# lrm2017/Fastest_Image_Pattern_Matching

Measured on AMD Instinct MI355X. Metric: template matches/sec + ms/search, 4024×3036 src ±180°; HBM GB/s vs roofline, higher is better.
Workload: dtype u8

## Files before the change

### fastest_image_pattern_matching_amd/_lib.py

```python
from __future__ import annotations

import ctypes as C
import os
import subprocess

_HERE = os.path.dirname(os.path.abspath(__file__))
LIB_PATH = os.path.join(_HERE, "lib", "libfpm_hip.so")
CSRC = os.path.join(_HERE, "csrc")

FPM_OK = 0
FPM_E_INVALID_ARG = -1
FPM_E_NOT_LEARNED = -2
FPM_E_SIZE = -3
FPM_E_DEVICE = -4
FPM_E_CAPACITY = -5
FPM_E_INTERNAL = -6

(FMT_GRAY8, FMT_BGR8, FMT_RGB8, FMT_BGRA8, FMT_RGBA8, FMT_BGR8_PLANAR, FMT_RGB8_PLANAR) = range(7)
FMT_COUNT = 7

(K_PYR, K_TOP_WARP, K_TOP_NCC, K_TOP_NMS, K_CAND_INIT, K_ROI_TABLES, K_ROI_WARP, K_ROI_CORR, K_ROI_EVAL, K_ROI_SMALL,
 K_CAND_STEP, K_TOP_MAP, K_NOT, K_PATCH, K_COMPARE, K_LEARN) = range(16)
KERNEL_NAMES = ["pyr_down", "top_warp", "top_ncc", "top_nms", "cand_init", "roi_tables", "roi_warp", "roi_corr",
                "roi_eval", "roi_small", "cand_step", "top_map", "bitwise_not", "patch_warp", "patch_compare"]
# ... 84 lines not shown
class AlignResult(C.Structure):

    _fields_ = [("lt_x", C.c_float), ("lt_y", C.c_float), ("angle", C.c_double), ("ssd_start", C.c_int64),
                ("ssd", C.c_int64), ("n_used", C.c_int64), ("evals", C.c_int32), ("best_eval", C.c_int32),
                ("flags", C.c_int32), ("reserved", C.c_int32)]


class Blob(C.Structure):

    _fields_ = [(n, C.c_int32) for n in ("hit", "seed", "area", "x0", "y0", "x1", "y1", "max_value")] + \
               [(n, C.c_int64) for n in ("sum_value", "sum_x", "sum_y")]


class BlobSummary(C.Structure):

    _fields_ = [("fg_pixels", C.c_int64)] + \
               [(n, C.c_int32) for n in ("n_components", "n_blobs", "n_returned", "largest_area", "flags", "reserved")]


class RoiRecord(C.Structure):

    _fields_ = [("score", C.c_float), ("mx", C.c_int32), ("my", C.c_int32), ("on_border", C.c_int32),
                ("vec", C.c_float * 9)]


class Peak(C.Structure):

    _fields_ = [("x", C.c_int32), ("y", C.c_int32), ("score", C.c_float)]


PEAKS_STATS_CALL, PEAKS_STATS_JOB = 8, 4
PEAKS_RAN_BLOCKS, PEAKS_RAN_NMS, PEAKS_RAN_FAST, PEAKS_RAN_GREEDY = 1, 2, 4, 8
TOP_MAPS_STATS = 8
TOP_FUSED_STATS = 8
TOP_FORM_EXACT16, TOP_FORM_EXACT14, TOP_FORM_SMALL, TOP_FORM_LARGE = 0, 1, 2, 3

_P = C.c_void_p
_U8P = C.POINTER(C.c_uint8)
SIGNATURES = {
    "fpm_params_default": (None, [C.POINTER(Params)]),
    "fpm_abi_version": (C.c_int, []),
    "fpm_create": (C.c_int, [C.c_int, C.POINTER(_P)]),
    "fpm_destroy": (C.c_int, [_P]),
    "fpm_last_error": (C.c_char_p, [_P]),
    "fpm_set_params": (C.c_int, [_P, C.POINTER(Params)]),
    "fpm_get_params": (C.c_int, [_P, C.POINTER(Params)]),
    "fpm_learn": (C.c_int, [_P, _U8P, C.c_int32, C.c_int32, C.c_size_t]),
    "fpm_clear_pattern": (C.c_int, [_P]),
    "fpm_is_learned": (C.c_int, [_P]),
    "fpm_match": (C.c_int, [_P, _U8P, C.c_int32, C.c_int32, C.c_size_t, C.POINTER(Result), C.c_int32,
                            C.POINTER(C.c_int32), C.POINTER(C.c_double)]),
    "fpm_stage_sources": (C.c_int, [_P, C.POINTER(_U8P), C.c_int32, C.c_int32, C.c_int32, C.c_size_t]),
    "fpm_stage_sources_device": (C.c_int, [_P, C.POINTER(_P), C.c_int32, C.c_int32, C.c_int32, C.c_size_t, C.c_size_t,
                                           C.c_int32, _P]),
    "fpm_match_device": (C.c_int, [_P, _P, C.c_int32, C.c_int32, C.c_size_t, C.c_size_t, C.c_int32, _P,
                                   C.POINTER(Result), C.c_int32, C.POINTER(C.c_int32), C.POINTER(C.c_double)]),
    "fpm_match_staged": (C.c_int, [_P, C.POINTER(Result), C.c_int32, C.POINTER(C.c_int32)]),
    "fpm_match_staged_launch": (C.c_int, [_P]),
    "fpm_match_staged_finish": (C.c_int, [_P, C.POINTER(Result), C.c_int32, C.POINTER(C.c_int32)]),
    "fpm_op_pyr_down": (C.c_int, [_P, _U8P, C.c_int32, C.c_int32, C.c_size_t, _U8P, C.c_size_t]),
    "fpm_op_pyr_down2": (C.c_int, [_P, _U8P, C.c_int32, C.c_int32, C.c_size_t, _U8P, C.c_size_t, _U8P, C.c_size_t,
                                   C.c_int32, C.c_int32]),
    "fpm_op_bitwise_not": (C.c_int, [_P, _U8P, C.c_int32, C.c_int32, C.c_size_t, _U8P, C.c_size_t]),
    "fpm_op_to_gray": (C.c_int, [_P, _P, C.c_int32, C.c_int32, C.c_size_t, C.c_size_t, C.c_int32, C.c_int32, _U8P,
                                 C.c_size_t]),
    "fpm_op_warp_affine": (C.c_int, [_P, _U8P, C.c_int32, C.c_int32, C.c_size_t, C.POINTER(C.c_double), _U8P,
                                     C.c_int32, C.c_int32, C.c_size_t, C.c_int32]),
# ... 144 lines not shown
```

### fastest_image_pattern_matching_amd/csrc/fpm_engine.hip

```cpp
#include <hip/hip_runtime.h>

#include <algorithm>
#include <array>
#include <cfloat>
#include <chrono>
#include <cmath>
#include <cstddef>
#include <cstdio>
#include <cstdlib>
#include <cstring>
#include <new>
#include <random>
#include <string>
#include <vector>

#include "../../include/fpm.h"
#include "fpm_host.h"
#include "fpm_kernels.h"
#include "fpm_model.h"

using namespace fpm;

namespace {

// ... 753 lines not shown
    hipStream_t st = ctx->stream;
    const SrcLevel& top = ctx->src[L];
    const TmplLevel& tt = ctx->tmpl[L];
    {
        const int64_t bytes = (int64_t)P.nang * top.w * top.h;
        ProfScope ps(ctx, FPM_K_TOP_WARP, bytes * S);
        launch_warp(P.d_jobs.as<WarpJob>(P.off_warp), J, P.max_canvas, st, P.d_livecnt.as<int32_t>(), P.nzero);
    }
    {
        int64_t bytes = 0;
        for (int a = 0; a < P.nang; ++a) bytes += 4LL * P.map_w[a] * P.map_h[a];
        ProfScope ps(ctx, FPM_K_TOP_NCC, bytes * S);
        if (ncc_tile_fits(tt.w, tt.h)) {
            int mw = 0, mh = 0;
            for (int a = 0; a < P.nang; ++a) { mw = std::max(mw, P.map_w[a]); mh = std::max(mh, P.map_h[a]); }
            launch_ncc_tile(P.d_jobs.as<NccJob>(P.off_ncc), J, mw, mh, tt.w, tt.h, st);
        } else {
            launch_ncc_map(P.d_jobs.as<NccJob>(P.off_ncc), J, P.max_map, tt.w * tt.h, st);
        }
    }
}

size_t plan_top_fused_lds(const fpm_ctx* ctx, size_t* need = nullptr) {
    const Plan& P = ctx->plan;
    const TmplLevel& tt = ctx->tmpl[P.L];
    if (need) *need = 0;
    if (P.by_block || !ncc_tile_fits(tt.w, tt.h) || P.S * P.nang <= 0) return 0;
    size_t lds = 0;
    for (int a = 0; a < P.nang; ++a) lds = std::max(lds, top_fused_lds(P.top[a].bw, P.top[a].bh, tt.w, tt.h));
    if (need) *need = lds;
    return lds > top_fused_lds_limit() ? 0 : lds;
}

void plan_top_choice(const fpm_ctx* ctx, size_t* fused_lds, bool* use_mma) {
    const Plan& P = ctx->plan;
    const char* top_env = getenv("FPM_TOP_FUSED");
    const int top_mode = top_env ? atoi(top_env) : -1;
    *fused_lds = 0;
    if (top_mode != 0 && (P.S * P.nang >= kTopFusedMinJobs || top_mode == 1)) *fused_lds = plan_top_fused_lds(ctx);
    const char* mma_env = getenv("FPM_TOP_MMA");
    *use_mma = P.top_mma && (*fused_lds == 0 || (mma_env && atoi(mma_env) == 1));
    if (*use_mma) *fused_lds = 0;
}

NmsArgs plan_nms_args(const fpm_ctx* ctx) {
    const Plan& P = ctx->plan;
    const TmplLevel& tt = ctx->tmpl[P.L];
    NmsArgs na{};
    na.jobs = P.d_jobs.as<NmsJob>(P.off_nms);
    na.peaks = P.d_peaks.as<Peak>();
    na.counts = P.d_counts.as<int32_t>();
    na.tw = tt.w; na.th = tt.h; na.cap = P.cap; na.by_block = P.by_block ? 1 : 0;
    na.mfc = ctx->prm.semantics == FPM_SEMANTICS_MFC ? 1 : 0;
    na.thr = P.layer_score[P.L]; na.overlap = ctx->prm.max_overlap;
    na.lds_blocks = 0;
    na.cand = nullptr; na.cand_cnt = nullptr; na.cand_cap = 0; na.cand_lds = 0; na.stamps = nullptr;
    na.skey = nullptr; na.sdone = nullptr;
    return na;
}

int enqueue_search(fpm_ctx* ctx) {
    Plan& P = ctx->plan;
    const int L = P.L, S = P.S, J = S * P.nang;
    const int stop = P.stop;
    hipStream_t st = ctx->stream;
    uint8_t* dsrc = ctx->d_src.as<uint8_t>();
    const SrcLevel& top = ctx->src[L];
    P.step_layers = 0;
    P.top_lists = false;
    size_t fused_lds = 0;
    bool use_mma = false;
    plan_top_choice(ctx, &fused_lds, &use_mma);
    int32_t* live[2] = {P.d_live.as<int32_t>(), P.d_live.as<int32_t>() + P.C};
    int32_t* livecnt = P.d_livecnt.as<int32_t>();
    CandInitArgs ca;
    ca.peaks = P.d_peaks.as<Peak>();
    ca.counts = P.d_counts.as<int32_t>();
    ca.angles = P.d_top.as<TopAngle>();
    ca.top_nodes = P.d_topn.as<AngleNode>();
    ca.state = P.d_state.as<CandState>();
    ca.live = live[0];
    ca.live_count = livecnt + 0;
    ca.nang = P.nang; ca.cap = P.cap; ca.total = P.C;
    ca.center = P.center;
    ca.refine = L > stop ? (L - 1 == stop ? 2 : 1) : 0;
    bool cand_fused = false;
    const bool top_init = fused_lds > 0 && P.cap <= kNmsInitCap && (size_t)J * P.cap == (size_t)P.C;
    const bool pyr_zero = (top_init && L >= 1) || use_mma;
    enqueue_pyramid(ctx, pyr_zero);
    NmsArgs na = plan_nms_args(ctx);
    if (fused_lds > 0) {
        int64_t bytes = (int64_t)P.nang * top.w * top.h;
        for (int a = 0; a < P.nang; ++a) bytes += 4LL * P.map_w[a] * P.map_h[a];
        ProfScope ps(ctx, FPM_K_TOP_NCC, bytes * S);
        launch_top_fused(P.d_jobs.as<WarpJob>(P.off_warp), P.d_jobs.as<NccJob>(P.off_ncc), na, J, fused_lds,
                         pyr_zero ? nullptr : P.d_livecnt.as<int32_t>(), pyr_zero ? 0 : P.nzero, st,
                         top_init ? &ca : nullptr, P.d_jobs.as<int32_t>(P.off_order), false);
        cand_fused = top_init;
    }
    if (use_mma) {
        const int mdim = P.nmax.max_map_dim;
        const long mpx = P.nmax.max_map_px;
        TopMmaArgs ta = P.tma;
        {
            ProfScope ps(ctx, FPM_K_TOP_NCC, (int64_t)S * P.nang * top.w * top.h);
            ta.mode = 0;
            launch_top_mma(ta, st);
        }
        const bool ci_ok = !P.by_block && P.cap <= kNmsInitCap && (size_t)J * P.cap == (size_t)P.C;
        NmsArgs ga = na;
        ga.cand = P.d_ncand.as<int32_t>(); ga.cand_val = P.d_tcandv.as<float>();
        ga.cand_cnt = ta.cand_cnt; ga.cand_cap = P.tcand_cap;
        ga.reset_untaken = P.by_block ? 1 : 0;
        {
            ProfScope ps(ctx, FPM_K_TOP_NMS, 0);
            launch_top_greedy(ga, J, P.max_cells, st, ci_ok ? &ca : nullptr);
        }
        P.top_lists = true;
        {
            ProfScope ps(ctx, FPM_K_TOP_MAP, 0);
            ta.mode = 1;
            launch_top_mma(ta, st);
        }
        {
            ProfScope ps(ctx, FPM_K_TOP_NMS, 0);
            NmsArgs fa = na;
            fa.cand = ga.cand; fa.cand_cnt = ga.cand_cnt; fa.cand_cap = P.tcand_cap;
            if (P.by_block) {
                fa.skey = (uint64_t*)(P.d_livecnt.as<int32_t>() + P.off_skey);
                fa.sdone = P.d_livecnt.as<int32_t>() + P.off_skey + 6 * J;
// ... 3205 lines not shown

int fpm_op_top_fused(fpm_ctx* ctx, int32_t* n_sources, int32_t* n_angles, int64_t* map_floats, int32_t* cap,
                     int32_t* geom, int32_t geom_cap, float* maps, int64_t maps_cap, fpm_peak* peaks, int32_t* counts,
                     fpm_peak* dump_peaks, int32_t* dump_counts, int64_t peak_slots, int32_t* stats) {
    if (!ctx) return FPM_E_INVALID_ARG;
    if (!ctx->learned) { ctx->err = "template not learned"; return FPM_E_NOT_LEARNED; }
    if (ctx->pending) { ctx->err = "a search is in flight (fpm_match_staged_finish first)"; return FPM_E_INVALID_ARG; }
    if (ctx->S <= 0 || !ctx->staged || !ctx->src_valid) { ctx->err = "top fused: no staged sources"; return FPM_E_INVALID_ARG; }
    const bool sizing = !geom && !maps && !peaks && !counts && !dump_peaks && !dump_counts;
    if (geom_cap < 0 || maps_cap < 0 || peak_slots < 0 ||
        (!sizing && (!geom || !maps || !peaks || !counts || !dump_peaks || !dump_counts))) {
        ctx->err = "bad top fused arguments";
        return FPM_E_INVALID_ARG;
    }
    HIP_TRY(hipSetDevice(ctx->device));
    struct ProfOff {
        fpm_ctx* c; bool was;
        explicit ProfOff(fpm_ctx* x) : c(x), was(x->prof) { c->prof = false; }
        ~ProfOff() { c->prof = was; }
    } prof_off(ctx);
    int rc = build_plan(ctx);
    if (rc != FPM_OK) return rc;
    Plan& P = ctx->plan;
    const int S = P.S, nang = P.nang, J = S * nang;
    std::vector<size_t> dense_off(nang);
    size_t dense = 0;
    for (int a = 0; a < nang; ++a) { dense_off[a] = dense; dense += (size_t)P.map_w[a] * P.map_h[a]; }
    if (n_sources) *n_sources = S;
    if (n_angles) *n_angles = nang;
    if (map_floats) *map_floats = (int64_t)dense;
    if (cap) *cap = P.cap;
    size_t need = 0;
    const size_t lds = plan_top_fused_lds(ctx, &need);
    if (stats) {
        size_t chosen = 0;
        bool use_mma = false;
        plan_top_choice(ctx, &chosen, &use_mma);
        std::fill(stats, stats + FPM_TOP_FUSED_STATS, 0);
        stats[0] = (int32_t)need;
        stats[1] = (int32_t)top_fused_static_lds(false);
        stats[2] = (int32_t)top_fused_lds_limit();
        stats[3] = top_fused_grid(J);
        stats[4] = J;
        stats[5] = P.cap;
        stats[6] = chosen > 0 ? 1 : 0;
        stats[7] = (int32_t)top_fused_static_lds(true);
    }
    if (lds == 0 && J > 0) {
        ctx->err = "top fused: the plan cannot take the fused form (block mode, the template level or the LDS limit)";
        return FPM_E_SIZE;
    }
    if (sizing) return FPM_OK;
    const size_t slots = (size_t)J * P.cap;
    if (geom_cap < nang || (uint64_t)maps_cap < (uint64_t)dense * S || (uint64_t)peak_slots < (uint64_t)slots) {
        ctx->err = "top fused: output capacity below the sizing call's";
        return FPM_E_CAPACITY;
    }
    for (int a = 0; a < nang; ++a) {
        geom[4 * a + 0] = P.top[a].bw; geom[4 * a + 1] = P.top[a].bh;
        geom[4 * a + 2] = P.map_w[a]; geom[4 * a + 3] = P.map_h[a];
    }
    if (J <= 0) return FPM_OK;
    hipStream_t st = ctx->stream;
    const size_t o_peaks[2] = {0, round_up(sizeof(Peak) * slots, (size_t)256)};
    const size_t o_counts[2] = {2 * o_peaks[1], 2 * o_peaks[1] + round_up(sizeof(int32_t) * J, (size_t)256)};
    HIP_TRY(ctx->d_op_b.ensure(o_counts[1] + sizeof(int32_t) * J));
    fpm_peak* hp_out[2] = {peaks, dump_peaks};
    int32_t* hc_out[2] = {counts, dump_counts};
    std::vector<Peak> hp[2];
    for (int v = 0; v < 2; ++v) {
        hp[v].resize(slots);
        for (size_t k = 0; k < slots; ++k) {
            Peak& q = hp[v][k];
            q.x = hp_out[v][k].x; q.y = hp_out[v][k].y; q.score = hp_out[v][k].score; q.pad = 0;
        }
        HIP_TRY(hipMemcpyAsync(ctx->d_op_b.as<char>(o_peaks[v]), hp[v].data(), sizeof(Peak) * slots, hipMemcpyHostToDevice, st));
        HIP_TRY(hipMemcpyAsync(ctx->d_op_b.as<char>(o_counts[v]), hc_out[v], sizeof(int32_t) * J, hipMemcpyHostToDevice, st));
    }
    rc = apply_polarity(ctx);
    if (rc != FPM_OK) return rc;
    HIP_TRY(hipMemsetAsync(P.d_map.p, 0xff, sizeof(float) * P.map_floats * S, st));
    enqueue_pyramid(ctx, false);
    for (int v = 0; v < 2; ++v) {
        NmsArgs na = plan_nms_args(ctx);
        na.peaks = ctx->d_op_b.as<Peak>(o_peaks[v]);
        na.counts = ctx->d_op_b.as<int32_t>(o_counts[v]);
        launch_top_fused(P.d_jobs.as<WarpJob>(P.off_warp), P.d_jobs.as<NccJob>(P.off_ncc), na, J, lds,
                         P.d_livecnt.as<int32_t>(), P.nzero, st, nullptr, P.d_jobs.as<int32_t>(P.off_order), v == 1);
        HIP_TRY(hipGetLastError());
    }
    std::vector<float> hm(P.map_floats * S);
    HIP_TRY(hipMemcpyAsync(hm.data(), P.d_map.p, sizeof(float) * hm.size(), hipMemcpyDeviceToHost, st));
    for (int v = 0; v < 2; ++v) {
        HIP_TRY(hipMemcpyAsync(hp[v].data(), ctx->d_op_b.as<char>(o_peaks[v]), sizeof(Peak) * slots, hipMemcpyDeviceToHost, st));
        HIP_TRY(hipMemcpyAsync(hc_out[v], ctx->d_op_b.as<char>(o_counts[v]), sizeof(int32_t) * J, hipMemcpyDeviceToHost, st));
    }
    HIP_TRY(hipStreamSynchronize(st));
    for (int s = 0; s < S; ++s)
        for (int a = 0; a < nang; ++a)
            std::copy_n(hm.data() + P.map_floats * s + P.map_off[a], (size_t)P.map_w[a] * P.map_h[a],
                        maps + dense * s + dense_off[a]);
    for (int v = 0; v < 2; ++v)
        for (size_t k = 0; k < slots; ++k) {
            fpm_peak& p = hp_out[v][k];
            const Peak& q = hp[v][k];
            p.x = q.x; p.y = q.y; p.score = q.score;
        }
    return FPM_OK;
}

int fpm_profile_enable(fpm_ctx* ctx, int32_t enable) {
    if (!ctx) return FPM_E_INVALID_ARG;
    ctx->prof = enable != 0;
    return FPM_OK;
}

int fpm_profile_reset(fpm_ctx* ctx) {
    if (!ctx) return FPM_E_INVALID_ARG;
    for (auto& k : ctx->kp) { k.ms = 0; k.launches = 0; k.bytes = 0; k.used = 0; }
    return FPM_OK;
}
// ... 19 lines not shown
```

### fastest_image_pattern_matching_amd/csrc/fpm_kernels.h

```cpp
#pragma once
#include <hip/hip_runtime.h>
#include <stdint.h>

#include "fpm_geom.h"

namespace fpm {

struct WarpJob {
    const uint8_t* src;
    uint8_t* dst;
    int32_t sw, sh, sp;
    int32_t dw, dh, dp;
    int32_t border;
    int32_t pad;
    double M[6];
};

struct NccJob {
    const uint8_t* img;
    const uint8_t* tmpl;
    float* out;
    int32_t iw, ih, ip;
    int32_t tw, th, tp;
    int32_t ow, oh;
// ... 270 lines not shown
    uint64_t* acc;
    uint32_t slack_off;
    int32_t nlv, nchunks;
    TmplPrepLevel lv[kTmplPrepMaxLevels];
};
bool launch_tmpl_prep(const TmplPrepArgs& a, hipStream_t st);
void launch_ncc_map(const NccJob* jobs, int njobs, int max_out, int tmpl_bytes, hipStream_t st);
bool ncc_tile_fits(int tw, int th);
void launch_ncc_tile(const NccJob* jobs, int njobs, int max_ow, int max_oh, int tw, int th, hipStream_t st);
constexpr int kNmsCandCap = 8192;
constexpr int kNmsInitCap = 128;
enum { kNmsRanBlocks = 1, kNmsRanNms = 2, kNmsRanFast = 4, kNmsRanGreedy = 8 };
struct NmsLaunchInfo {
    uint32_t kernels;
    int32_t lds_blocks;
    int32_t cand_lds;
    int32_t greedy_cap;
    int32_t blk_lds;
};
void launch_nms(const NmsArgs& a, int njobs, int max_blocks, int max_map_dim, int max_cells, hipStream_t st,
                int max_items = 0, const CandInitArgs* ci = nullptr, long max_map_px = -1,
                NmsLaunchInfo* info = nullptr);
int nms_block_items(int mw, int mh, int tw, int th, int mfc);
struct NmsMaxima {
    int max_blocks = 0, max_map_dim = 0, max_cells = 0, max_items = 0;
    long max_map_px = 0;
};
int nms_maxima_add(NmsMaxima& m, int mw, int mh, int tw, int th, int by_block, int mfc);
int nms_plain_form(int blk_lds, int cap, long n);
void launch_cand_init(const CandInitArgs& a, hipStream_t st);
size_t top_fused_lds(int bw, int bh, int tw, int th);
size_t top_fused_lds_limit();
constexpr int kTopFusedMinJobs = 256;
void launch_top_fused(const WarpJob* wjobs, const NccJob* njobs, const NmsArgs& a, int njobs_n, size_t lds,
                      int32_t* zero, int nzero, hipStream_t st, const CandInitArgs* ci, const int32_t* order,
                      bool dump);
size_t top_fused_static_lds(bool dump);
int top_fused_grid(int njobs_n);
struct TopUnit { int32_t job, x0, y0, y1; };
constexpr int kTopMmaMaxSw = 192;
struct TopMmaArgs {
    const WarpJob* wjobs;
    const NccJob* njobs;
    const TopUnit* units;
    int32_t nunits;
    const uint8_t* bfrag;
    int32_t nq, R;
    int32_t tw, th, area;
    uint32_t tsum;
    int32_t sw;
    int32_t cp;
    int32_t rr;
    int32_t ct, rt;
    int32_t o_colt, o_rowt, o_bf, o_ft;
    int32_t nqm;
    int32_t mode;
    int32_t prefilter;
    float thrK, E;
    double thr, mean, norm, inv_area;
    int32_t* cand;
    float* cand_val;
    int32_t* cand_cnt;
    int32_t cand_cap;
};
size_t top_mma_lds(const TopMmaArgs& a);
void top_mma_layout(TopMmaArgs& a, int sw, int max_rows);
bool top_mma_fits(int tw, int th);
void launch_top_mma(const TopMmaArgs& a, hipStream_t st);
enum { kTopFormExact16 = 0, kTopFormExact14 = 1, kTopFormSmall = 2, kTopFormLarge = 3 };
// ... 29 lines not shown
```

### fastest_image_pattern_matching_amd/csrc/fpm_kernels.hip

```cpp
#include <float.h>
#include <stdio.h>
#include <stdlib.h>
#include <limits.h>

#include <map>
#include <mutex>
#include <type_traits>
#include <utility>

#include "../../include/fpm.h"
#include "fpm_kernels.h"
#include "fpm_model.h"
#include "fpm_rrect.h"

static void ensure_lds_attr(const void* fn, size_t bytes) {
    if (bytes <= 65536) return;
    int dev = 0;
    (void)hipGetDevice(&dev);
    static std::mutex mu;
    static std::map<std::pair<int, const void*>, size_t> done;
    std::lock_guard<std::mutex> lock(mu);
    size_t& cur = done[std::make_pair(dev, fn)];
    if (bytes <= cur) return;
    (void)hipFuncSetAttribute(fn, hipFuncAttributeMaxDynamicSharedMemorySize, (int)bytes);
// ... 5 lines not shown
__device__ __forceinline__ int rint_i(double v) { return (int)__builtin_rint(v); }
__device__ __forceinline__ int sat_s16(int v) { return v < -32768 ? -32768 : (v > 32767 ? 32767 : v); }
__device__ __forceinline__ int reflect101(int p, int n) {
    if (n == 1) return 0;
    while (p < 0 || p >= n) p = p < 0 ? -p : 2 * n - 2 - p;
    return p;
}
__device__ __forceinline__ double dmax0(double a) { return a < 0.0 ? 0.0 : a; }
__device__ __forceinline__ double dmin(double a, double b) { return b < a ? b : a; }

__device__ __forceinline__ int warp_tap(const uint8_t* __restrict__ src, int sw, int sh, int sp, int X, int Y,
                                        int cval) {
    const int sx = sat_s16(X >> kInterBits), sy = sat_s16(Y >> kInterBits);
    const int fx = X & (kInterTab - 1), fy = Y & (kInterTab - 1);
    const int w0 = (kInterTab - fy) * (kInterTab - fx) * 32, w1 = (kInterTab - fy) * fx * 32;
    const int w2 = fy * (kInterTab - fx) * 32, w3 = fy * fx * 32;
    int v0, v1, v2, v3;
    if ((unsigned)sx < (unsigned)(sw > 1 ? sw - 1 : 0) && (unsigned)sy < (unsigned)(sh > 1 ? sh - 1 : 0)) {
        const uint8_t* p = src + (size_t)sy * sp + sx;
        v0 = p[0]; v1 = p[1]; v2 = p[sp]; v3 = p[sp + 1];
    } else if (sx >= sw || sx + 1 < 0 || sy >= sh || sy + 1 < 0) {
        return cval;
    } else {
        const bool x0 = sx >= 0 && sx < sw, x1 = sx + 1 >= 0 && sx + 1 < sw;
        const bool y0 = sy >= 0 && sy < sh, y1 = sy + 1 >= 0 && sy + 1 < sh;
        const uint8_t* r0 = src + (size_t)sy * sp;
        const uint8_t* r1 = r0 + sp;
        v0 = x0 && y0 ? r0[sx] : cval;
        v1 = x1 && y0 ? r0[sx + 1] : cval;
        v2 = x0 && y1 ? r1[sx] : cval;
        v3 = x1 && y1 ? r1[sx + 1] : cval;
    }
    return (v0 * w0 + v1 * w1 + v2 * w2 + v3 * w3 + (1 << 14)) >> 15;
}

__device__ __forceinline__ float ccoeff(double num, double wsum, double wsq, double mean0, double tnorm,
                                        double inv_area) {
    double wndMean2 = 0, wndSum2 = 0, t;
    t = wsum;
    wndMean2 += t * t;
    num -= t * mean0;
    wndMean2 *= inv_area;
    t = wsq;
    wndSum2 += t;
    const double diff2 = dmax0(wndSum2 - wndMean2);
    if (diff2 <= dmin(0.5, (double)(10 * FLT_EPSILON) * wndSum2))
        t = 0;
    else
        t = __builtin_sqrt(diff2) * tnorm;
    if (__builtin_fabs(num) < t)
        num /= t;
    else if (__builtin_fabs(num) < t * 1.125)
        num = num > 0 ? 1 : -1;
    else
        num = 0;
    return (float)num;
}

__device__ __forceinline__ int xcd_remap(int b, int n) {
    const int q = n >> 3, r = n & 7, x = b & 7;
    return (x < r ? x * (q + 1) : r * (q + 1) + (x - r) * q) + (b >> 3);
}
struct XcdSplit { int lo, hi, k, nk; };
__device__ __forceinline__ XcdSplit xcd_split(int n) {
    const int G = gridDim.x, b = blockIdx.x, x = b & 7, q = G >> 3, r = G & 7;
    const int nk = q + (x < r ? 1 : 0);
// ... 1730 lines not shown
    const int job = id / a.cap, r = id - job * a.cap, ang = job % a.nang;
    CandState s;
    s.lt = f2(0.f, 0.f);
    s.node = ang;
    s.alive = 0;
    s.reached0 = 0;
    s.pad = 0;
    if (r < a.counts[job]) {
        const Peak pk = a.peaks[id];
        const F2 pt = f2((float)pk.x - a.angles[ang].tx, (float)pk.y - a.angles[ang].ty);
        s.lt = rotate_pt(pt, a.center, a.top_nodes[ang].cn, a.top_nodes[ang].sn);
        if (a.refine) {
            s.alive = 1;
            s.reached0 = mark_reached0;
            const int slot = atomicAdd(a.live_count, 1);
            a.live[slot] = id;
        }
    }
    a.state[id] = s;
}

void launch_cand_init(const CandInitArgs& a, hipStream_t st) {
    if (a.total <= 0) return;
    CandInitArgs b = a;
    const int mark = a.refine == 2 ? 1 : 0;
    if (b.refine) b.refine = 1;
    hipLaunchKernelGGL(k_cand_init, dim3((a.total + 255) / 256), dim3(256), 0, st, b, mark);
}

constexpr int kTopThreads = 256;
template <bool DUMP>
__device__ __forceinline__ void top_fused_job(int job, const WarpJob* __restrict__ wjobs,
                                              const NccJob* __restrict__ njobs, const NmsArgs& a,
                                              const CandInitArgs& ci, int ci_mode, uint32_t* tf_lds, float* sv,
                                              int* si, Peak* spk, int* sbase_p) {
    int& sbase = *sbase_p;
    const int tid = threadIdx.x;
    const WarpJob& w = wjobs[job];
    const NccJob& j = njobs[job];
    const int dw = w.dw, dh = w.dh, cpw = ((dw + 3) >> 2) + 1;
    const int tw = j.tw, th = j.th, ntw = (tw + 3) >> 2, ow = j.ow, oh = j.oh, n = ow * oh;
    if (n <= 0) {
        if (tid == 0) a.counts[job] = 0;
        if (ci_mode) cand_init_job(ci, ci_mode, job, 0, spk, &sbase);
        return;
    }
    uint32_t* Cw = tf_lds;
    float* Mp = (float*)(Cw + dh * cpw);
    uint32_t* Tw = (uint32_t*)(Mp + n);
    uint32_t* Mw = Tw + th * ntw;
    int32_t* tab = (int32_t*)(Mw + ntw);

    for (int x = tid; x < dw; x += kTopThreads) {
        tab[x] = rint_i(w.M[0] * x * kAbScale);
        tab[dw + x] = rint_i(w.M[3] * x * kAbScale);
    }
    for (int y = tid; y < dh; y += kTopThreads) {
        tab[2 * dw + y] = rint_i((w.M[1] * y + w.M[2]) * kAbScale) + kRoundDelta;
        tab[2 * dw + dh + y] = rint_i((w.M[4] * y + w.M[5]) * kAbScale) + kRoundDelta;
    }
    __syncthreads();
    for (int i = tid; i < dh * cpw; i += kTopThreads) {
        const int y = i / cpw, k = i - y * cpw;
        const int X0 = tab[2 * dw + y], Y0 = tab[2 * dw + dh + y];
        uint32_t word = 0;
        for (int b = 0; b < 4; ++b) {
            const int x = 4 * k + b;
            if (x >= dw) break;
            const int ad = tab[x], bd = tab[dw + x];
            const int X = (X0 + ad) >> (kAbBits - kInterBits), Y = (Y0 + bd) >> (kAbBits - kInterBits);
            word |= (uint32_t)warp_tap(w.src, w.sw, w.sh, w.sp, X, Y, w.border) << (8 * b);
        }
        Cw[i] = word;
    }
    for (int i = tid; i < th * ntw; i += kTopThreads) {
        const int r = i / ntw, k = i - r * ntw;
        uint32_t t = 0;
        for (int b = 0; b < 4; ++b)
            if (4 * k + b < tw) t |= (uint32_t)j.tmpl[(size_t)r * j.tp + 4 * k + b] << (8 * b);
        Tw[i] = t;
    }
    if (tid < ntw) {
        uint32_t m = 0;
        for (int b = 0; b < 4; ++b)
            if (4 * tid + b < tw) m |= 1u << (8 * b);
        Mw[tid] = m;
    }
    __syncthreads();
    const int ngx = (ow + 3) >> 2;
    for (int it = tid; it < oh * ngx; it += kTopThreads) {
        const int y = it / ngx, q = it - y * ngx;
        uint32_t d[4] = {0, 0, 0, 0}, s1[4] = {0, 0, 0, 0}, s2[4] = {0, 0, 0, 0};
        for (int r = 0; r < th; ++r) {
            const uint32_t* ir = Cw + (y + r) * cpw + q;
            const uint32_t* tr = Tw + r * ntw;
            uint32_t w0 = ir[0];
            for (int k = 0; k < ntw; ++k) {
                const uint32_t w1 = ir[k + 1], t = tr[k], m = Mw[k], mff = m * 0xffu;
                const uint32_t sh[4] = {w0, __builtin_amdgcn_alignbyte(w1, w0, 1),
                                        __builtin_amdgcn_alignbyte(w1, w0, 2), __builtin_amdgcn_alignbyte(w1, w0, 3)};
#pragma unroll
                for (int u = 0; u < 4; ++u) {
                    d[u] = __builtin_amdgcn_udot4(t, sh[u], d[u], false);
                    s1[u] = __builtin_amdgcn_udot4(m, sh[u], s1[u], false);
                    s2[u] = __builtin_amdgcn_udot4(sh[u] & mff, sh[u], s2[u], false);
                }
                w0 = w1;
            }
        }
#pragma unroll
        for (int u = 0; u < 4; ++u) {
            const int x = 4 * q + u;
            if (x >= ow) break;
            const double num = (double)(float)(double)(uint64_t)d[u];
            Mp[y * ow + x] = j.equal1 ? 1.f : ccoeff(num, (double)s1[u], (double)s2[u], j.mean, j.norm, j.inv_area);
        }
    }
    __syncthreads();
    if constexpr (DUMP)
        for (int k = tid; k < n; k += kTopThreads) j.out[k] = Mp[k];
    Peak* out = a.peaks + (size_t)job * a.cap;
    const double ov = a.overlap;
    float v = -INFINITY;
    int i = INT_MAX;
    for (int k = tid; k < n; k += kTopThreads) { const float x = Mp[k]; if (x > v) { v = x; i = k; } }
    wg_argmax(v, i, sv, si);
    if ((double)v < a.thr) {
        if (tid == 0) a.counts[job] = 0;
        if (ci_mode) cand_init_job(ci, ci_mode, job, 0, spk, &sbase);
        return;
    }
    int cnt = 0;
    int px = i % ow, py = i / ow;
    if (tid == 0) {
        out[0].x = px; out[0].y = py; out[0].score = v;
        if (ci_mode) { spk[0].x = px; spk[0].y = py; spk[0].score = v; }
    }
    ++cnt;
    for (int itn = 0; itn < a.cap - 1; ++itn) {
        const int sx = (int)(px - a.tw * (1 - ov)), sy = (int)(py - a.th * (1 - ov));
        const int rw = (int)(2 * a.tw * (1 - ov)), rh = (int)(2 * a.th * (1 - ov));
        if (rw > 0 && rh > 0) {
            const int x1 = sx > 0 ? sx : 0, y1 = sy > 0 ? sy : 0;
            const int x2 = min(sx + rw - 1, ow - 1), y2 = min(sy + rh - 1, oh - 1);
            const int cw = x2 - x1 + 1, ch = y2 - y1 + 1;
            if (cw > 0 && ch > 0)
                for (int k = tid; k < cw * ch; k += kTopThreads) Mp[(y1 + k / cw) * ow + x1 + k % cw] = -1.f;
        }
        __syncthreads();
        v = -INFINITY;
        i = INT_MAX;
        for (int k = tid; k < n; k += kTopThreads) { const float x = Mp[k]; if (x > v) { v = x; i = k; } }
        wg_argmax(v, i, sv, si);
        if ((double)v < a.thr) break;
        px = i % ow;
        py = i / ow;
        if (tid == 0) {
            out[cnt].x = px; out[cnt].y = py; out[cnt].score = v;
            if (ci_mode) { spk[cnt].x = px; spk[cnt].y = py; spk[cnt].score = v; }
        }
        ++cnt;
    }
    if (tid == 0) a.counts[job] = cnt;
    if (ci_mode) cand_init_job(ci, ci_mode, job, cnt, spk, &sbase);
}

template <bool DUMP>
__global__ __launch_bounds__(kTopThreads) void k_top_fused(const WarpJob* __restrict__ wjobs,
                                                           const NccJob* __restrict__ njobs,
                                                           NmsArgs a, int32_t* zero, int nzero,
                                                           CandInitArgs ci, int ci_mode, const int32_t* order,
                                                           int njobs_n) {
    extern __shared__ __attribute__((aligned(16))) uint32_t tf_lds[];
    __shared__ float sv[kTopThreads / 64];
    __shared__ int si[kTopThreads / 64];
    __shared__ Peak spk[kNmsInitCap];
    __shared__ int sbase;
    if (blockIdx.x == 0)
        for (int i = threadIdx.x; i < nzero; i += kTopThreads) zero[i] = 0;
    for (int k = blockIdx.x; k < njobs_n; k += gridDim.x) {
        if (k != (int)blockIdx.x) __syncthreads();
        top_fused_job<DUMP>(order ? order[k] : k, wjobs, njobs, a, ci, ci_mode, tf_lds, sv, si, spk, &sbase);
    }
}

size_t top_fused_lds(int bw, int bh, int tw, int th) {
    const int cpw = ((bw + 3) >> 2) + 1, ntw = (tw + 3) >> 2;
    const size_t map = (size_t)std::max(bw - tw + 1, 0) * std::max(bh - th + 1, 0);
    return 4 * ((size_t)bh * cpw + map + (size_t)th * ntw + ntw + 2 * ((size_t)bw + bh));
}

size_t top_fused_lds_limit() {
    int dev = 0;
    (void)hipGetDevice(&dev);
    static std::mutex mu;
    static std::map<int, size_t> lim;
    std::lock_guard<std::mutex> lock(mu);
    auto it = lim.find(dev);
    if (it != lim.end()) return it->second;
    hipFuncAttributes fa{};
    size_t stat = 8192;
    if (hipFuncGetAttributes(&fa, (const void*)k_top_fused<false>) == hipSuccess) stat = fa.sharedSizeBytes;
    const size_t l = stat < 65536 ? 65536 - stat : 0;
    lim[dev] = l;
    return l;
}

size_t top_fused_static_lds(bool dump) {
    hipFuncAttributes fa{};
    const void* f = dump ? (const void*)k_top_fused<true> : (const void*)k_top_fused<false>;
    return hipFuncGetAttributes(&fa, f) == hipSuccess ? fa.sharedSizeBytes : 0;
}

int top_fused_grid(int njobs_n) {
    const char* gte = getenv("FPM_GRID_TOP");
    const int grid_cap = gte && atoi(gte) > 0 ? atoi(gte) : 0;
    return grid_cap > 0 && njobs_n > grid_cap ? grid_cap : njobs_n;
}

void launch_top_fused(const WarpJob* wjobs, const NccJob* njobs, const NmsArgs& a, int njobs_n, size_t lds,
                      int32_t* zero, int nzero, hipStream_t st, const CandInitArgs* ci, const int32_t* order,
                      bool dump) {
    if (njobs_n <= 0) return;
    if (dump) {
        static std::once_flag once;
        std::call_once(once, [] {
            const size_t sp = top_fused_static_lds(false), sd = top_fused_static_lds(true);
            if (sp == 0 || sp != sd) {
                std::fprintf(stderr, "fpm: k_top_fused<true> and <false> differ in static LDS (%zu, %zu)\n", sd, sp);
                std::abort();
            }
        });
    }
    CandInitArgs cz{};
    const bool fuse = ci && a.cap <= kNmsInitCap;
    const int mode = !fuse ? 0 : (ci->refine == 0 ? 1 : (ci->refine == 2 ? 3 : 2));
    if (fuse && zero && nzero > 0 && mode != 1) {
        std::fprintf(stderr, "fpm: launch_top_fused contract violated (counter zeroing with candidate-init mode %d)\n",
                     mode);
        std::abort();
    }
    const int grid = top_fused_grid(njobs_n);
    if (dump)
        hipLaunchKernelGGL(k_top_fused<true>, dim3(grid), dim3(kTopThreads), lds, st, wjobs, njobs, a, zero, nzero,
                           fuse ? *ci : cz, mode, order, njobs_n);
    else
        hipLaunchKernelGGL(k_top_fused<false>, dim3(grid), dim3(kTopThreads), lds, st, wjobs, njobs, a, zero, nzero,
                           fuse ? *ci : cz, mode, order, njobs_n);
}

constexpr int ROI_T = 32;
constexpr int ROI_FT = 4096;
constexpr int kFtPitch = 68;
constexpr int kTabShift = 6;
constexpr int kTabFrac = kAbBits + kTabShift;
constexpr int kTapShift = kTabFrac - kInterBits;
constexpr uint32_t kRoiFlip = 0x80808080u;

__host__ __device__ inline int roi_pitch_calc(int tw) {
    const int need_a = tw + 6 + 16, need_b = 64 * ((tw + 63) / 64) + 22;
    int q = ((need_a > need_b ? need_a : need_b) + 15) / 16;
    if ((q & 1) == 0) ++q;
    return q * 16;
}
int roi_pitch_for(int tw) { return roi_pitch_calc(tw); }
int roi_bands(int th) { return (th + 2 * kMmaRows - 1) / (2 * kMmaRows); }
int roi_tab_rows(int th) { return (th + 6 + ROI_T - 1) / ROI_T * ROI_T; }
__host__ __device__ inline int roi_tab_row_pos(int y) { return (y & ~31) | ((y & 7) << 2) | ((y >> 3) & 3); }
size_t roi_tiles_bytes(int tw, int th) {
    return (size_t)((tw + 6 + ROI_T - 1) / ROI_T) * ((th + 6 + ROI_T - 1) / ROI_T) * ROI_T * ROI_T;
}

__host__ __device__ inline int tmpl_lds_pitch(int tp8) {
    int q = tp8 / 16;
    if ((q & 1) == 0) ++q;
    return q * 16;
}

size_t roi_corr_lds(int roi_pitch) {
    constexpr int src_rows = 2 * kMmaRows + 6;
    return (size_t)src_rows * roi_pitch +
// ... 3487 lines not shown
```

### fastest_image_pattern_matching_amd/matcher.py

```python
from __future__ import annotations

import ctypes as C
import os
from dataclasses import dataclass
from typing import List, Sequence, Tuple

import numpy as np

from . import _lib as L


@dataclass
class SingleTargetMatch:

    ptLT: Tuple[float, float]
    ptRT: Tuple[float, float]
    ptRB: Tuple[float, float]
    ptLB: Tuple[float, float]
    ptCenter: Tuple[float, float]
    dMatchedAngle: float
    dMatchScore: float

    @staticmethod
    def from_c(r: "L.Result") -> "SingleTargetMatch":
# ... 1235 lines not shown
        S, nang, cap, dense = ns.value, na.value, lc.value, mf.value
        geom = np.zeros((max(nang, 1), 4), np.int32)
        out = {}
        if form in (0, 1):
            flat = np.zeros(max(S * dense, 1), np.float32)
            call(geom.ctypes.data_as(IP), nang, flat.ctypes.data_as(FP), S * dense, None, None, None, 0)
            offs = np.concatenate([[0], np.cumsum(geom[:nang, 2].astype(np.int64) * geom[:nang, 3])])
            out["maps"] = [[flat[s * dense + offs[a]:s * dense + offs[a + 1]].reshape(geom[a, 3], geom[a, 2])
                            for a in range(nang)] for s in range(S)]
        else:
            cnt = np.zeros(max(S * nang, 1), np.int32)
            idx = np.zeros(max(S * nang * cap, 1), np.int32)
            val = np.zeros(max(S * nang * cap, 1), np.float32)
            call(geom.ctypes.data_as(IP), nang, None, 0, cnt.ctypes.data_as(IP), idx.ctypes.data_as(IP),
                 val.ctypes.data_as(FP), S * nang * cap)
            out["counts"] = cnt[:S * nang].reshape(S, nang)
            out["index"] = idx[:S * nang * cap].reshape(S, nang, cap)
            out["value"] = val[:S * nang * cap].reshape(S, nang, cap)
        out["geom"] = geom[:nang]
        out["stats"] = dict(top_mma=int(st[0]), list_cap=int(st[1]), sw=int(st[2]), run=int(st[3]), nunits=int(st[4]),
                            form=int(st[5]), map_grid=int(st[6]), by_block=int(st[7]))
        return out

    TOP_FUSED_FILL = (-7, -7, -7.0)

    def top_fused(self):
        IP, FP, PP = C.POINTER(C.c_int32), C.POINTER(C.c_float), C.POINTER(L.Peak)
        ns, na, cp, mf = C.c_int32(), C.c_int32(), C.c_int32(), C.c_int64()
        st = np.zeros(L.TOP_FUSED_STATS, np.int32)
        self._push()

        def stats():
            return dict(lds=int(st[0]), static_lds=int(st[1]), lds_limit=int(st[2]), grid=int(st[3]), jobs=int(st[4]),
                        cap=int(st[5]), search_takes_it=int(st[6]), dump_static_lds=int(st[7]))

        def call(geom, gcap, maps, mcap, pk, cnt, dpk, dcnt, slots):
            rc = self._check(self._lib.fpm_op_top_fused(
                self._ctx, C.byref(ns), C.byref(na), C.byref(mf), C.byref(cp), geom, gcap, maps, mcap, pk, cnt, dpk, dcnt,
                slots, st.ctypes.data_as(IP)), "top_fused")
            if rc != L.FPM_OK:
                e = ValueError(f"fpm_op_top_fused failed with {rc}: {self.last_error()}")
                e.rc = rc
                e.stats = stats()
                raise e

        call(None, 0, None, 0, None, None, None, None, 0)
        S, nang, cap, dense = ns.value, na.value, cp.value, mf.value
        geom = np.zeros((max(nang, 1), 4), np.int32)
        flat = np.zeros(max(S * dense, 1), np.float32)
        pk = [np.zeros(max(S * nang * cap, 1), PEAK_DTYPE) for _ in range(2)]
        cnt = [np.full(max(S * nang, 1), self.TOP_FUSED_FILL[0], np.int32) for _ in range(2)]
        for p in pk:
            p["x"], p["y"], p["score"] = self.TOP_FUSED_FILL
        call(geom.ctypes.data_as(IP), nang, flat.ctypes.data_as(FP), S * dense, pk[0].ctypes.data_as(PP),
             cnt[0].ctypes.data_as(IP), pk[1].ctypes.data_as(PP), cnt[1].ctypes.data_as(IP), S * nang * cap)
        offs = np.concatenate([[0], np.cumsum(geom[:nang, 2].astype(np.int64) * geom[:nang, 3])])
        return dict(geom=geom[:nang], stats=stats(),
                    maps=[[flat[s * dense + offs[a]:s * dense + offs[a + 1]].reshape(geom[a, 3], geom[a, 2])
                           for a in range(nang)] for s in range(S)],
                    peaks=pk[0][:S * nang * cap].reshape(S, nang, cap), counts=cnt[0][:S * nang].reshape(S, nang),
                    dump_peaks=pk[1][:S * nang * cap].reshape(S, nang, cap),
                    dump_counts=cnt[1][:S * nang].reshape(S, nang))

    def overlap_filter(self, corners, scores, max_overlap: float, device: bool = True):
        c = np.ascontiguousarray(corners, np.float32).reshape(-1, 6)
        sc = np.ascontiguousarray(scores, np.float64).ravel()
        n = c.shape[0]
# ... 47 lines not shown
```

### include/fpm.h

```cpp
#ifndef FPM_H_
#define FPM_H_

#include <stddef.h>
#include <stdint.h>

#ifdef __cplusplus
extern "C" {
#endif

#define FPM_ABI_VERSION 11

#define FPM_OK 0
#define FPM_E_INVALID_ARG (-1)
#define FPM_E_NOT_LEARNED (-2)
#define FPM_E_SIZE (-3)
#define FPM_E_DEVICE (-4)
#define FPM_E_CAPACITY (-5)
#define FPM_E_INTERNAL (-6)

#define FPM_SEMANTICS_QT 0
#define FPM_SEMANTICS_MFC 1

typedef struct fpm_params {
    int32_t max_pos;
// ... 224 lines not shown
int fpm_op_ncc_map(fpm_ctx* ctx, const uint8_t* src, int32_t w, int32_t h, size_t src_stride,
                   int32_t layer, int32_t fold, float* out);
int fpm_op_overlap_filter(fpm_ctx* ctx, const float* corners, const double* scores, int32_t n, double max_overlap,
                          int32_t mode, int32_t* keep, int32_t* n_keep, int32_t* stats);
typedef struct fpm_roi_record {
    float score;
    int32_t mx, my;
    int32_t on_border;
    float vec[9];
} fpm_roi_record;
int fpm_op_refine(fpm_ctx* ctx, const uint8_t* const* levels, int32_t count, int32_t w, int32_t h, size_t stride,
                  int32_t layer, const float* lt, const double* angles, int32_t n, int32_t n3, int32_t fold,
                  int32_t round_rois, fpm_roi_record* rec, uint8_t* roi_pixels, int32_t* pixels_written);
typedef struct fpm_peak {
    int32_t x, y;
    float score;
} fpm_peak;
#define FPM_PEAKS_MAX_PIXELS (1 << 26)
#define FPM_PEAKS_MAX_SLOTS (1 << 24)
#define FPM_PEAKS_STATS_CALL 8
#define FPM_PEAKS_STATS_JOB 4
int fpm_op_peaks(fpm_ctx* ctx, const float* const* maps, const int32_t* mw, const int32_t* mh, int32_t n_maps,
                 int32_t tw, int32_t th, int32_t cap, int32_t by_block, int32_t mfc, double thr, double overlap,
                 int32_t form, int32_t list_cap, uint32_t list_seed, fpm_peak* peaks, int32_t* counts,
                 int32_t* stats);
#define FPM_TOP_MAPS_STATS 8
#define FPM_TOP_FORM_EXACT16 0
#define FPM_TOP_FORM_EXACT14 1
#define FPM_TOP_FORM_SMALL 2
#define FPM_TOP_FORM_LARGE 3
int fpm_op_top_maps(fpm_ctx* ctx, int32_t form, double thr, int32_t* n_sources, int32_t* n_angles, int64_t* map_floats,
                    int32_t* list_cap, int32_t* geom, int32_t geom_cap, float* maps, int64_t maps_cap,
                    int32_t* list_count, int32_t* list_index, float* list_value, int64_t list_slots, int32_t* stats);
#define FPM_TOP_FUSED_STATS 8
int fpm_op_top_fused(fpm_ctx* ctx, int32_t* n_sources, int32_t* n_angles, int64_t* map_floats, int32_t* cap,
                     int32_t* geom, int32_t geom_cap, float* maps, int64_t maps_cap, fpm_peak* peaks, int32_t* counts,
                     fpm_peak* dump_peaks, int32_t* dump_counts, int64_t peak_slots, int32_t* stats);
int fpm_template_info(const fpm_ctx* ctx, int32_t* levels, int32_t* border_color);
int fpm_template_level(const fpm_ctx* ctx, int32_t level, int32_t* w, int32_t* h, double* mean,
                       double* norm, double* inv_area, int32_t* result_equal1, uint8_t* pixels,
                       size_t stride);

int fpm_search_stats(const fpm_ctx* ctx, int64_t* stats, int32_t cap);
int fpm_search_bytes(const fpm_ctx* ctx, int64_t* b_pyr, int64_t* b_top, int64_t* b_ref);

#define FPM_K_PYR 0
#define FPM_K_TOP_WARP 1
#define FPM_K_TOP_NCC 2
#define FPM_K_TOP_NMS 3
#define FPM_K_CAND_INIT 4
#define FPM_K_ROI_TABLES 5
#define FPM_K_ROI_WARP 6
#define FPM_K_ROI_CORR 7
#define FPM_K_ROI_EVAL 8
#define FPM_K_ROI_SMALL 9
#define FPM_K_CAND_STEP 10
#define FPM_K_TOP_MAP 11
#define FPM_K_NOT 12
#define FPM_K_PATCH 13
#define FPM_K_COMPARE 14
#define FPM_K_LEARN 15
#define FPM_K_COUNT 16
int fpm_profile_enable(fpm_ctx* ctx, int32_t enable);
int fpm_profile_reset(fpm_ctx* ctx);
int fpm_profile_get(const fpm_ctx* ctx, int32_t kernel, double* total_ms, int64_t* launches,
                    int64_t* bytes);
int fpm_profile_last(const fpm_ctx* ctx, double* device_ms, double* host_ms, double* call_ms);
// ... 7 lines not shown
```

Before: 36500.

## Stage top pyramid level in LDS and skip NCC scoring below integer bound

The fused top-level kernel now copies the top source level into LDS as padded pairs of bytes, so bilinear warping reads from LDS with udot4 instead of gathering from global memory, when the level fits in the map area. It also adds an integer/float correlation upper-bound test that skips the double-precision ccoeff evaluation and writes -2 for positions that cannot pass the threshold. Launch bounds now request 6 blocks per CU. The intent is to cut both global gather latency and double-precision arithmetic, at the cost of an extra LDS fill per job, register pressure from the occupancy hint, and reliance on the bound being conservative.

```diff
diff --git a/fastest_image_pattern_matching_amd/_lib.py b/fastest_image_pattern_matching_amd/_lib.py
--- a/fastest_image_pattern_matching_amd/_lib.py
+++ b/fastest_image_pattern_matching_amd/_lib.py
@@ -140,7 +140,7 @@
 PEAKS_STATS_CALL, PEAKS_STATS_JOB = 8, 4
 PEAKS_RAN_BLOCKS, PEAKS_RAN_NMS, PEAKS_RAN_FAST, PEAKS_RAN_GREEDY = 1, 2, 4, 8
 TOP_MAPS_STATS = 8
-TOP_FUSED_STATS = 8
+TOP_FUSED_STATS = 10
 TOP_FORM_EXACT16, TOP_FORM_EXACT14, TOP_FORM_SMALL, TOP_FORM_LARGE = 0, 1, 2, 3
 
 _P = C.c_void_p
diff --git a/fastest_image_pattern_matching_amd/csrc/fpm_engine.hip b/fastest_image_pattern_matching_amd/csrc/fpm_engine.hip
--- a/fastest_image_pattern_matching_amd/csrc/fpm_engine.hip
+++ b/fastest_image_pattern_matching_amd/csrc/fpm_engine.hip
@@ -809,6 +809,28 @@
     return lds > top_fused_lds_limit() ? 0 : lds;
 }
 
+TopFusedOpts plan_top_fused_opts(const fpm_ctx* ctx, int* copy_angles = nullptr) {
+    const Plan& P = ctx->plan;
+    const TmplLevel& tt = ctx->tmpl[P.L];
+    const SrcLevel& top = ctx->src[P.L];
+    TopFusedOpts o{};
+    int fits = 0;
+    for (int a = 0; a < P.nang; ++a) fits += top_fused_level_fits(top.w, top.h, P.map_w[a], P.map_h[a]) ? 1 : 0;
+    o.level_copy = fits > 0 && ctx->border >= 0 && ctx->border <= 255 ? 1 : 0;
+    if (copy_angles) *copy_angles = o.level_copy ? fits : 0;
+    const double thr = P.layer_score[P.L];
+    o.area = (uint32_t)(tt.w * tt.h);
+    if (o.area <= 258 && thr > 0.01 && !tt.equal1 && tt.px.size() == (size_t)o.area) {
+        TopMmaArgs A{};
+        A.area = (int32_t)o.area;
+        top_mma_thresholds(A, thr, tt);
+        o.thrK = A.thrK; o.E = A.E;
+        for (uint8_t v : tt.px) o.tsum += v;
+        o.bound = 1;
+    }
+    return o;
+}
+
 void plan_top_choice(const fpm_ctx* ctx, size_t* fused_lds, bool* use_mma) {
     const Plan& P = ctx->plan;
     const char* top_env = getenv("FPM_TOP_FUSED");
@@ -872,7 +894,7 @@
         ProfScope ps(ctx, FPM_K_TOP_NCC, bytes * S);
         launch_top_fused(P.d_jobs.as<WarpJob>(P.off_warp), P.d_jobs.as<NccJob>(P.off_ncc), na, J, fused_lds,
                          pyr_zero ? nullptr : P.d_livecnt.as<int32_t>(), pyr_zero ? 0 : P.nzero, st,
-                         top_init ? &ca : nullptr, P.d_jobs.as<int32_t>(P.off_order), false);
+                         top_init ? &ca : nullptr, P.d_jobs.as<int32_t>(P.off_order), false, plan_top_fused_opts(ctx));
         cand_fused = top_init;
     }
     if (use_mma) {
@@ -4144,6 +4166,8 @@
     if (cap) *cap = P.cap;
     size_t need = 0;
     const size_t lds = plan_top_fused_lds(ctx, &need);
+    int copy_angles = 0;
+    const TopFusedOpts opts = plan_top_fused_opts(ctx, &copy_angles);
     if (stats) {
         size_t chosen = 0;
         bool use_mma = false;
@@ -4157,6 +4181,8 @@
         stats[5] = P.cap;
         stats[6] = chosen > 0 ? 1 : 0;
         stats[7] = (int32_t)top_fused_static_lds(true);
+        stats[8] = copy_angles;
+        stats[9] = opts.bound;
     }
     if (lds == 0 && J > 0) {
         ctx->err = "top fused: the plan cannot take the fused form (block mode, the template level or the LDS limit)";
@@ -4198,7 +4224,8 @@
         na.peaks = ctx->d_op_b.as<Peak>(o_peaks[v]);
         na.counts = ctx->d_op_b.as<int32_t>(o_counts[v]);
         launch_top_fused(P.d_jobs.as<WarpJob>(P.off_warp), P.d_jobs.as<NccJob>(P.off_ncc), na, J, lds,
-                         P.d_livecnt.as<int32_t>(), P.nzero, st, nullptr, P.d_jobs.as<int32_t>(P.off_order), v == 1);
+                         P.d_livecnt.as<int32_t>(), P.nzero, st, nullptr, P.d_jobs.as<int32_t>(P.off_order), v == 1,
+                         opts);
         HIP_TRY(hipGetLastError());
     }
     std::vector<float> hm(P.map_floats * S);
diff --git a/fastest_image_pattern_matching_amd/csrc/fpm_kernels.h b/fastest_image_pattern_matching_amd/csrc/fpm_kernels.h
--- a/fastest_image_pattern_matching_amd/csrc/fpm_kernels.h
+++ b/fastest_image_pattern_matching_amd/csrc/fpm_kernels.h
@@ -326,9 +326,20 @@
 size_t top_fused_lds(int bw, int bh, int tw, int th);
 size_t top_fused_lds_limit();
 constexpr int kTopFusedMinJobs = 256;
+struct TopFusedOpts {
+    int32_t level_copy;
+    int32_t bound;
+    float thrK, E;
+    uint32_t tsum, area;
+};
+constexpr int top_fused_level_pitch(int sw) { return (sw + 1 + 3) & ~3; }
+constexpr size_t top_fused_level_bytes(int sw, int sh) { return 2 * (size_t)top_fused_level_pitch(sw) * (size_t)(sh + 2); }
+constexpr bool top_fused_level_fits(int sw, int sh, int ow, int oh) {
+    return ow > 0 && oh > 0 && top_fused_level_bytes(sw, sh) <= 4 * (size_t)ow * (size_t)oh;
+}
 void launch_top_fused(const WarpJob* wjobs, const NccJob* njobs, const NmsArgs& a, int njobs_n, size_t lds,
                       int32_t* zero, int nzero, hipStream_t st, const CandInitArgs* ci, const int32_t* order,
-                      bool dump);
+                      bool dump, const TopFusedOpts& opts);
 size_t top_fused_static_lds(bool dump);
 int top_fused_grid(int njobs_n);
 struct TopUnit { int32_t job, x0, y0, y1; };
diff --git a/fastest_image_pattern_matching_amd/csrc/fpm_kernels.hip b/fastest_image_pattern_matching_amd/csrc/fpm_kernels.hip
--- a/fastest_image_pattern_matching_amd/csrc/fpm_kernels.hip
+++ b/fastest_image_pattern_matching_amd/csrc/fpm_kernels.hip
@@ -61,6 +61,17 @@
         v3 = x1 && y1 ? r1[sx + 1] : cval;
     }
     return (v0 * w0 + v1 * w1 + v2 * w2 + v3 * w3 + (1 << 14)) >> 15;
+}
+
+__device__ __forceinline__ int warp_tap_lds(const uint16_t* lv, int lp, int sw, int sh, int X, int Y) {
+    const int sx = sat_s16(X >> kInterBits), sy = sat_s16(Y >> kInterBits);
+    const int fx = X & (kInterTab - 1), fy = Y & (kInterTab - 1);
+    const bool in = (unsigned)(sx + 1) <= (unsigned)sw && (unsigned)(sy + 1) <= (unsigned)sh;
+    const int i0 = in ? (sy + 1) * lp + sx + 1 : 0, i1 = in ? i0 + lp : 0;
+    const uint32_t wx = (uint32_t)(kInterTab - fx) | (uint32_t)fx << 8;
+    const uint32_t r0 = __builtin_amdgcn_udot4((uint32_t)lv[i0], wx, 0u, false);
+    const uint32_t r1 = __builtin_amdgcn_udot4((uint32_t)lv[i1], wx, 0u, false);
+    return (int)(((r0 * (uint32_t)(kInterTab - fy) + r1 * (uint32_t)fy) * 32u + (1u << 14)) >> 15);
 }
 
 __device__ __forceinline__ float ccoeff(double num, double wsum, double wsq, double mean0, double tnorm,
@@ -1857,8 +1868,8 @@
 template <bool DUMP>
 __device__ __forceinline__ void top_fused_job(int job, const WarpJob* __restrict__ wjobs,
                                               const NccJob* __restrict__ njobs, const NmsArgs& a,
-                                              const CandInitArgs& ci, int ci_mode, uint32_t* tf_lds, float* sv,
-                                              int* si, Peak* spk, int* sbase_p) {
+                                              const CandInitArgs& ci, int ci_mode, const TopFusedOpts& o,
+                                              uint32_t* tf_lds, float* sv, int* si, Peak* spk, int* sbase_p) {
     int& sbase = *sbase_p;
     const int tid = threadIdx.x;
     const WarpJob& w = wjobs[job];
@@ -1884,19 +1895,68 @@
         tab[2 * dw + y] = rint_i((w.M[1] * y + w.M[2]) * kAbScale) + kRoundDelta;
         tab[2 * dw + dh + y] = rint_i((w.M[4] * y + w.M[5]) * kAbScale) + kRoundDelta;
     }
+    const int lp = top_fused_level_pitch(w.sw);
+    const bool lvl = o.level_copy && top_fused_level_fits(w.sw, w.sh, ow, oh);
+    if (lvl) {
+        uint32_t* Lw = (uint32_t*)Mp;
+        const int lpi = lp >> 2;
+        const uint32_t b1 = (uint32_t)(w.border & 0xff), b4 = b1 * 0x01010101u;
+        const bool al = ((((uintptr_t)w.src) | (uintptr_t)(uint32_t)w.sp) & 3) == 0;
+        for (int i = tid; i < lpi * (w.sh + 2); i += kTopThreads) {
+            const int r = i / lpi, k = i - r * lpi;
+            const int y = r - 1, x = 4 * k;
+            uint32_t v = b4, prev = b1;
+            if ((unsigned)y < (unsigned)w.sh) {
+                const uint8_t* p = w.src + (size_t)y * w.sp + x;
+                if (k > 0 && x - 1 < w.sw) prev = p[-1];
+                const int nb = w.sw - x;
+                if (nb > 0) {
+                    if (al && x + 4 <= w.sp) {
+                        v = *(const uint32_t*)p;
+                    } else {
+                        v = 0;
+                        for (int b = 0; b < 4 && b < nb; ++b) v |= (uint32_t)p[b] << (8 * b);
+                    }
+                    if (nb < 4) {
+                        const uint32_t keep = (1u << (8 * nb)) - 1u;
+                        v = (v & keep) | (b4 & ~keep);
+                    }
+                }
+            }
+            Lw[2 * i] = prev | (v & 0xffu) << 8 | (v & 0xffffu) << 16;
+            Lw[2 * i + 1] = ((v >> 8) & 0xffffu) | (v >> 16) << 16;
+        }
+    }
     __syncthreads();
-    for (int i = tid; i < dh * cpw; i += kTopThreads) {
-        const int y = i / cpw, k = i - y * cpw;
-        const int X0 = tab[2 * dw + y], Y0 = tab[2 * dw + dh + y];
-        uint32_t word = 0;
-        for (int b = 0; b < 4; ++b) {
-            const int x = 4 * k + b;
-            if (x >= dw) break;
-            const int ad = tab[x], bd = tab[dw + x];
-            const int X = (X0 + ad) >> (kAbBits - kInterBits), Y = (Y0 + bd) >> (kAbBits - kInterBits);
-            word |= (uint32_t)warp_tap(w.src, w.sw, w.sh, w.sp, X, Y, w.border) << (8 * b);
-        }
-        Cw[i] = word;
+    if (lvl) {
+        const uint16_t* lv = (const uint16_t*)Mp;
+        for (int i = tid; i < dh * cpw; i += kTopThreads) {
+            const int y = i / cpw, k = i - y * cpw;
+            const int X0 = tab[2 * dw + y], Y0 = tab[2 * dw + dh + y];
+            uint32_t word = 0;
+            for (int b = 0; b < 4; ++b) {
+                const int x = 4 * k + b;
+                if (x >= dw) break;
+                const int ad = tab[x], bd = tab[dw + x];
+                const int X = (X0 + ad) >> (kAbBits - kInterBits), Y = (Y0 + bd) >> (kAbBits - kInterBits);
+                word |= (uint32_t)warp_tap_lds(lv, lp, w.sw, w.sh, X, Y) << (8 * b);
+            }
+            Cw[i] = word;
+        }
+    } else {
+        for (int i = tid; i < dh * cpw; i += kTopThreads) {
+            const int y = i / cpw, k = i - y * cpw;
+            const int X0 = tab[2 * dw + y], Y0 = tab[2 * dw + dh + y];
+            uint32_t word = 0;
+            for (int b = 0; b < 4; ++b) {
+                const int x = 4 * k + b;
+                if (x >= dw) break;
+                const int ad = tab[x], bd = tab[dw + x];
+                const int X = (X0 + ad) >> (kAbBits - kInterBits), Y = (Y0 + bd) >> (kAbBits - kInterBits);
+                word |= (uint32_t)warp_tap(w.src, w.sw, w.sh, w.sp, X, Y, w.border) << (8 * b);
+            }
+            Cw[i] = word;
+        }
     }
     for (int i = tid; i < th * ntw; i += kTopThreads) {
         const int r = i / ntw, k = i - r * ntw;
@@ -1933,12 +1993,36 @@
                 w0 = w1;
             }
         }
-#pragma unroll
-        for (int u = 0; u < 4; ++u) {
-            const int x = 4 * q + u;
-            if (x >= ow) break;
-            const double num = (double)(float)(double)(uint64_t)d[u];
-            Mp[y * ow + x] = j.equal1 ? 1.f : ccoeff(num, (double)s1[u], (double)s2[u], j.mean, j.norm, j.inv_area);
+        uint32_t pm = 0xfu;
+        if constexpr (!DUMP) {
+            if (o.bound) {
+                pm = 0;
+#pragma unroll
+                for (int u = 0; u < 4; ++u) {
+                    const uint32_t dfi = o.area * s2[u] - s1[u] * s1[u];
+                    const float nfp =
+                        __builtin_fmaf((float)o.area, (float)d[u], -((float)s1[u] * (float)o.tsum)) + o.E;
+                    if (dfi != 0u && nfp > 0.f && nfp * nfp >= o.thrK * (float)dfi) pm |= 1u << u;
+                }
+            }
+        }
+        if (pm) {
+#pragma unroll
+            for (int u = 0; u < 4; ++u) {
+                const int x = 4 * q + u;
+                if (x >= ow) break;
+                const double num = (double)(float)(double)(uint64_t)d[u];
+                const float sc =
+                    j.equal1 ? 1.f : ccoeff(num, (double)s1[u], (double)s2[u], j.mean, j.norm, j.inv_area);
+                Mp[y * ow + x] = (pm >> u) & 1u ? sc : -2.f;
+            }
+        } else {
+#pragma unroll
+            for (int u = 0; u < 4; ++u) {
+                const int x = 4 * q + u;
+                if (x >= ow) break;
+                Mp[y * ow + x] = -2.f;
+            }
         }
     }
     __syncthreads();
@@ -1991,11 +2075,11 @@
 }
 
 template <bool DUMP>
-__global__ __launch_bounds__(kTopThreads) void k_top_fused(const WarpJob* __restrict__ wjobs,
+__global__ __launch_bounds__(kTopThreads, 6) void k_top_fused(const WarpJob* __restrict__ wjobs,
                                                            const NccJob* __restrict__ njobs,
                                                            NmsArgs a, int32_t* zero, int nzero,
                                                            CandInitArgs ci, int ci_mode, const int32_t* order,
-                                                           int njobs_n) {
+                                                           int njobs_n, TopFusedOpts o) {
     extern __shared__ __attribute__((aligned(16))) uint32_t tf_lds[];
     __shared__ float sv[kTopThreads / 64];
     __shared__ int si[kTopThreads / 64];
@@ -2005,7 +2089,7 @@
         for (int i = threadIdx.x; i < nzero; i += kTopThreads) zero[i] = 0;
     for (int k = blockIdx.x; k < njobs_n; k += gridDim.x) {
         if (k != (int)blockIdx.x) __syncthreads();
-        top_fused_job<DUMP>(order ? order[k] : k, wjobs, njobs, a, ci, ci_mode, tf_lds, sv, si, spk, &sbase);
+        top_fused_job<DUMP>(order ? order[k] : k, wjobs, njobs, a, ci, ci_mode, o, tf_lds, sv, si, spk, &sbase);
     }
 }
 
@@ -2045,7 +2129,7 @@
 
 void launch_top_fused(const WarpJob* wjobs, const NccJob* njobs, const NmsArgs& a, int njobs_n, size_t lds,
                       int32_t* zero, int nzero, hipStream_t st, const CandInitArgs* ci, const int32_t* order,
-                      bool dump) {
+                      bool dump, const TopFusedOpts& opts) {
     if (njobs_n <= 0) return;
     if (dump) {
         static std::once_flag once;
@@ -2068,10 +2152,10 @@
     const int grid = top_fused_grid(njobs_n);
     if (dump)
         hipLaunchKernelGGL(k_top_fused<true>, dim3(grid), dim3(kTopThreads), lds, st, wjobs, njobs, a, zero, nzero,
-                           fuse ? *ci : cz, mode, order, njobs_n);
+                           fuse ? *ci : cz, mode, order, njobs_n, opts);
     else
         hipLaunchKernelGGL(k_top_fused<false>, dim3(grid), dim3(kTopThreads), lds, st, wjobs, njobs, a, zero, nzero,
-                           fuse ? *ci : cz, mode, order, njobs_n);
+                           fuse ? *ci : cz, mode, order, njobs_n, opts);
 }
 
 constexpr int ROI_T = 32;
diff --git a/fastest_image_pattern_matching_amd/matcher.py b/fastest_image_pattern_matching_amd/matcher.py
--- a/fastest_image_pattern_matching_amd/matcher.py
+++ b/fastest_image_pattern_matching_amd/matcher.py
@@ -1291,7 +1291,8 @@
 
         def stats():
             return dict(lds=int(st[0]), static_lds=int(st[1]), lds_limit=int(st[2]), grid=int(st[3]), jobs=int(st[4]),
-                        cap=int(st[5]), search_takes_it=int(st[6]), dump_static_lds=int(st[7]))
+                        cap=int(st[5]), search_takes_it=int(st[6]), dump_static_lds=int(st[7]), copy_angles=int(st[8]),
+                        bound=int(st[9]))
 
         def call(geom, gcap, maps, mcap, pk, cnt, dpk, dcnt, slots):
             rc = self._check(self._lib.fpm_op_top_fused(
diff --git a/include/fpm.h b/include/fpm.h
--- a/include/fpm.h
+++ b/include/fpm.h
@@ -280,7 +280,7 @@
 int fpm_op_top_maps(fpm_ctx* ctx, int32_t form, double thr, int32_t* n_sources, int32_t* n_angles, int64_t* map_floats,
                     int32_t* list_cap, int32_t* geom, int32_t geom_cap, float* maps, int64_t maps_cap,
                     int32_t* list_count, int32_t* list_index, float* list_value, int64_t list_slots, int32_t* stats);
-#define FPM_TOP_FUSED_STATS 8
+#define FPM_TOP_FUSED_STATS 10
 int fpm_op_top_fused(fpm_ctx* ctx, int32_t* n_sources, int32_t* n_angles, int64_t* map_floats, int32_t* cap,
                      int32_t* geom, int32_t geom_cap, float* maps, int64_t maps_cap, fpm_peak* peaks, int32_t* counts,
                      fpm_peak* dump_peaks, int32_t* dump_counts, int64_t peak_slots, int32_t* stats);
```

Measured after the change: 36920 (median of 6 runs). 1.01x the previous value.
